# lars-frogner/Impact

Measured on AMD Instinct MI355X. Metric: voxels stepped/sec + remesh tris/sec, 512^3 grid, 1/2/4/8 MI355X, higher is better.
Workload: dtype i8 voxels, f32 SDF/mesh arithmetic, f64 moments; 1 GPU; config-2 SDF asteroid x2.05 -> 502^3 grid = 512^3 stored voxels (32768 chunks); parallelism=single GPU, voxels_per_gpu=134217728, regions=1, triangles=1813104

## Files before the change

### impact_amd/csrc/derive.hip

```cpp
#include "device_common.hpp"
#include "chunk_passes.hpp"
#include "table_roles.hpp"
#include "many.hpp"

#ifndef IVX_POL_SWEEP_PLANES
#define IVX_POL_SWEEP_PLANES IVX_ST_WT
#endif
#ifndef IVX_DERIVE_WAVES
#define IVX_DERIVE_WAVES 6
#endif

namespace {

struct DeriveParams {
    uint32_t cx, cy, cz;
};

__device__ __forceinline__ uint32_t row_mask(uint4 s) {
    uint32_t w[4] = {s.x, s.y, s.z, s.w};
    uint32_t m = 0;
#pragma unroll
    for (int q = 0; q < 4; ++q) m |= ((((w[q] >> 7) & 0x01010101u) * 0x00204081u >> 21) & 0xFu) << (4 * q);
    return m;
}
// ... 8 lines not shown
    GridView g;
    ivx_chunk_info* info;
    uint32_t* bbox;
    uint32_t* mesh_counts;
    uint8_t* chunk_class;
    uint8_t* touch;
    uint32_t* rparent;
    uint32_t* work_counts;
    uint32_t* next_work_count;
    uint32_t* active_list;
    ivx_roles::PresetArgs preset;
    uint32_t defer_ghost, pad_;
    unsigned long long* tick;
};
__device__ __forceinline__ void chunk_settle(const GridView& g, const ChunkPreArgs& a, uint32_t chunk, const ivx_chunk_info& own) {
    const uint32_t gen = own.gen_kind;
    const bool solid = gen == KIND_UNIFORM;
    ivx_chunk_info rec = own;
    rec.kind = (uint8_t)gen;
    rec.flags = 0;
    rec.face_dist = solid ? 0x555 : 0;
    rec.uniform_type = solid ? (own.kind == KIND_NONUNIFORM ? g.type[(size_t)chunk * IVX_CHUNK_VOXELS] : own.uniform_type) : (uint8_t)0;
    rec.region_count = solid ? 1 : 0;
    rec.boundary_region_count = solid ? 1 : 0;
    a.info[chunk] = rec;
    a.bbox[chunk] = solid ? (0x80000000u | (15u << 4) | (15u << 12) | (15u << 20)) : 0u;
    a.mesh_counts[2 * chunk] = 0;
    a.mesh_counts[2 * chunk + 1] = 0;
    a.touch[chunk] = solid ? 7 : 0;
    if (solid) a.rparent[(size_t)chunk * 256] = chunk * 256u;
}
__device__ __forceinline__ void chunk_pre_body(const ChunkPreArgs& a, uint32_t bid, uint32_t) {
    const GridView& g = a.g;
    ivx_chunk_info* __restrict__ info = a.info;
    uint32_t* __restrict__ bbox = a.bbox;
    uint32_t* __restrict__ mesh_counts = a.mesh_counts;
    uint8_t* __restrict__ chunk_class = a.chunk_class;
    uint8_t* __restrict__ touch = a.touch;
    uint32_t* __restrict__ rparent = a.rparent;
    uint32_t* __restrict__ work_counts = a.work_counts;
    uint32_t* __restrict__ next_work_count = a.next_work_count;
    uint32_t* __restrict__ active_list = a.active_list;
    __shared__ uint32_t s_w[4];
    __shared__ uint32_t s_base;
    const uint32_t tid = threadIdx.x, lane = tid & 63u, wave = tid >> 6;
    ivx_roles::role_preset(a.preset, bid * 256u + tid);
    if (bid == 0 && tid == 0) next_work_count[0] = 0u;
    const uint32_t n_chunks = g.cx * g.cy * g.cz;
    const uint32_t chunk = bid * 256u + tid;
    const bool live = chunk < n_chunks;
    bool settled = false, pending = false;
    if (live) {
        const ivx_chunk_info own = info[chunk];
        const uint32_t gen = own.gen_kind;
// ... 135 lines not shown
    int8_t* sdf_rw;
    uint8_t* type_rw;
    uint8_t* flags_out;
    ivx_chunk_info* info;
    uint32_t* bbox;
    uint8_t* touch;
    uint16_t* signs;
    uint8_t* kface_out;
    const uint32_t* work_counts;
    uint32_t* active_list;
    const uint32_t* list_in;
    DeriveFused fz;
    uint32_t signs_type, x_part;
    DeriveBox box;
    unsigned long long* tick;
};
template <bool SIGNS>
__device__ __forceinline__ void derive_body(const DeriveArgs& a_, uint32_t bid_, uint32_t nb_) {
    const GridView& g = a_.g;
    int8_t* __restrict__ sdf_rw = a_.sdf_rw;
    uint8_t* __restrict__ type_rw = a_.type_rw;
    uint8_t* __restrict__ flags_out = a_.flags_out;
    ivx_chunk_info* __restrict__ info = a_.info;
    uint32_t* __restrict__ bbox = a_.bbox;
    uint8_t* __restrict__ touch = a_.touch;
    uint16_t* __restrict__ signs = a_.signs;
    uint8_t* __restrict__ kface_out = a_.kface_out;
    const uint32_t* __restrict__ work_counts = a_.work_counts;
    uint32_t* __restrict__ active_list = a_.active_list;
    const uint32_t* __restrict__ list_in = a_.list_in;
// ... 685 lines not shown
            ci_.flags = 0;
            ci_.face_dist = 0x555;
            ci_.uniform_type = (uint8_t)utype;
        } else {
            ci_.flags = 0;
            ci_.face_dist = 0;
        }
        info[chunk] = ci_;
    }
    IVX_TW(g, li, 5);
    ivx_wave_lds_sync();
    }
}
__global__ __launch_bounds__(256) __attribute__((amdgpu_waves_per_eu(IVX_DERIVE_WAVE_WAVES, 8))) void k_derive_wave(DeriveArgs a) {
    ivx_stage_stamp(a.tick);
    derive_wave_body(a);
}

struct ListRebuildArgs {
    GridView g;
    const ivx_chunk_info* info;
    uint32_t* work_counts;
    uint32_t* next_work_count;
    uint32_t* active_list;
    uint32_t* mesh_counts;
};
__device__ __forceinline__ void list_rebuild_body(const ListRebuildArgs& a, uint32_t bid, uint32_t) {
    const GridView& g = a.g;
    const ivx_chunk_info* __restrict__ info = a.info;
    uint32_t* __restrict__ work_counts = a.work_counts;
// ... 131 lines not shown
    g->planes_compact = 0;
    return IVX_OK;
}

ivx_roles::PresetArgs ivx_preset_args(ivx_grid* g, uint32_t groups) {
    const uint32_t n_groups = (g->n_chunks + 255u) / 256u;
    ivx_roles::PresetArgs a;
    a.groups = groups;
    a.rscalar = g->rscalar;
    a.sn_sums = g->group_sums + n_groups;
    a.n_sn = IVX_SN_GROUP_WORDS * n_groups;
    a.eval_count = g->samp_len ? g->samp_len + g->n_chunks : nullptr;
    return a;
}

int ivx_launch_step_preset(ivx_grid* g, uint32_t groups) {
    if (!groups) return IVX_OK;
    const ivx_roles::PresetArgs a = ivx_preset_args(g, groups);
    IVX_KLAUNCH(k_step_preset, dim3((a.n_sn + 255u) / 256u), dim3(256), 0, g->ctx->stream, a);
    IVX_HIP_CHECK(hipGetLastError());
    g->scratch_dirty &= ~groups;
    return IVX_OK;
}

#ifdef IVX_DERIVE_DEBUG
static void derive_debug_mask() {
    static bool done = false;
    if (done) return;
    done = true;
    const char* e = getenv("IVX_DERIVE_SKIP");
// ... 7 lines not shown
#endif
    GridView v = ivx_view(g);
    DeriveFused fz;
    fz.parts = parts;
    fz.x_off = g->x_off;
    fz.labels = g->llabel;
    fz.rparent = g->rparent;
    fz.rscalar = g->rscalar;
    fz.multi_list = g->ccl_scratch;
    fz.dens = g->dens_dev;
    fz.chunk_moments = g->chunk_moments;
    if ((parts & IVX_PART_REGIONS) && !(preset_groups & IVX_SCRATCH_REGIONS) && (g->scratch_dirty & IVX_SCRATCH_REGIONS))
        IVX_HIP_CHECK(ivx_memset_async(g->rscalar, 0, 16 * sizeof(uint32_t), g->ctx->stream));
    if (parts & IVX_PART_REGIONS) g->scratch_dirty |= IVX_SCRATCH_REGIONS;
    g->bbox_valid = 1;
    uint32_t* next_count = ivx_wc(g);
    g->wc_cur ^= 1u;
    const uint32_t roll = ((g->scratch_dirty & IVX_SCRATCH_EVAL) && g->samp_len) ? IVX_SCRATCH_EVAL_ROLL : 0u;
    ChunkPreArgs face_settle;
    {
        ChunkPreArgs pa;
        memset(&pa, 0, sizeof(pa));
        pa.g = v, pa.info = g->info, pa.bbox = g->chunk_bbox, pa.mesh_counts = g->chunk_counts, pa.chunk_class = g->chunk_class, pa.touch = g->chunk_touch;
        pa.rparent = g->rparent, pa.work_counts = ivx_wc(g), pa.next_work_count = next_count, pa.active_list = g->active_list;
        pa.preset = ivx_preset_args(g, preset_groups | roll);
        if (g->ghost_event && g->ghost_split && ivx_has_interior_planes(g)) pa.defer_ghost = 1u;
        const uint32_t blocks = (g->n_chunks + 255u) / 256u;
        pa.tick = g->timing.take(ivx_many_recording());
        if (!ivx_many_try(g->ctx, g, IVX_MK_CHUNK_PRE, blocks, pa)) IVX_KLAUNCH(k_chunk_pre, dim3(blocks), dim3(256), 0, g->ctx->stream, pa);
        face_settle = pa;
        face_settle.tick = nullptr;
    }
    g->scratch_dirty &= ~preset_groups;
    if (roll) g->scratch_dirty &= ~IVX_SCRATCH_EVAL;
    uint32_t derive_grid = ivx_list_grid(g);
    if (g->last_active) {
        const uint32_t per_round = (uint32_t)g->ctx->n_cu * 32u;
        const uint32_t each = (g->last_active + per_round / 2u) / per_round > 1u ? (g->last_active + per_round / 2u) / per_round : 1u;
        derive_grid = (g->last_active + each - 1u) / each;
        const uint32_t lo = (g->n_chunks + 255u) / 256u;
        if (derive_grid < lo) derive_grid = lo;
    }
    DeriveArgs da = derive_args(g, v, fz);
    if (g->signs_current) da.signs_type = (uint32_t)g->signs_type;
    uint32_t wave_grid;
    {
        const uint32_t per_round = (uint32_t)g->ctx->n_cu * 4u * IVX_DERIVE_WAVE_WAVES;
        const uint32_t n = g->last_active ? g->last_active : per_round;
        const uint32_t each = (n + per_round / 2u) / per_round > 1u ? (n + per_round / 2u) / per_round : 1u;
        wave_grid = ((n + each - 1u) / each + 3u) / 4u;
    }
    auto sweep = [&](uint32_t x_part) {
        da.x_part = x_part;
        da.tick = g->timing.take(ivx_many_recording());
        if (g->signs_current) {
            if (ivx_many_try(g->ctx, g, IVX_MK_DERIVE_SIGNS, derive_grid, da)) return;
            if (x_part == IVX_XPART_ALL && v.ghost_sdf[0] == nullptr && v.ghost_sdf[1] == nullptr)
                IVX_KLAUNCH(k_derive_wave, dim3(wave_grid), dim3(256), 0, g->ctx->stream, da);
            else
// ... 90 lines not shown
```

### impact_amd/csrc/ivx_api.hip

```cpp
#include <algorithm>
#include <array>
#include <functional>
#include <cmath>
#include <chrono>
#include <cstring>
#include <new>
#include <type_traits>
#include <vector>

#include "ivx_host.hpp"

static thread_local char g_error[512] = "";

void ivx_set_error(const char* fmt, ...) {
    va_list ap;
    va_start(ap, fmt);
    vsnprintf(g_error, sizeof(g_error), fmt, ap);
    va_end(ap);
}

namespace {

int ensure_host_scratch(ivx_grid* g, size_t bytes) {
    if (g->host_scratch_bytes >= bytes) return IVX_OK;
// ... 402 lines not shown
    if (which == 0 || which == 1 || which == 4) ivx_planes_touched(g);
    switch (which) {
        case 0: return g->sdf;
        case 1: return g->type;
        case 2: return g->flags;
        case 3: return g->llabel;
        case 4: return g->info;
        case 5: return g->rparent;
#ifdef IVX_WG_TRACE
        case 6: return g->chunk_moments;
#endif
        case 7: return g->samp_len;
        case 8: return g->samp_ops;
        case 10: return g->sn_hard;
        case 9: return ivx_sn_hard_count(g);
        default: return nullptr;
    }
}

int ivx_sdf_sample(ivx_grid* g, const ivx_sdf_processed_node* nodes, size_t n_nodes, uint32_t stack_size, const uint32_t grid_shape[3],
                   const float shifted_grid_center[3], uint8_t voxel_type) {
    IVX_REQUIRE(g && grid_shape && shifted_grid_center, IVX_ERR_INVALID, "ivx_sdf_sample: null argument");
    IVX_REQUIRE(n_nodes == 0 || nodes, IVX_ERR_INVALID, "ivx_sdf_sample: null node array");
    for (int d = 0; d < 3; ++d) {
        const uint32_t cap = (d == 0 ? g->gx : g->cc[d]) * 16u;
        IVX_REQUIRE(grid_shape[d] <= cap, IVX_ERR_INVALID, "ivx_sdf_sample: grid shape %u exceeds the chunk grid (%u voxels) along axis %d", grid_shape[d], cap, d);
    }
    int depth = 0, max_depth = 0;
    for (size_t i = 0; i < n_nodes; ++i) {
        const uint32_t k = nodes[i].kind;
// ... 688 lines not shown
```

### impact_amd/csrc/ivx_internal.hpp

```cpp
#pragma once
#include <hip/hip_runtime.h>

#include <cstdarg>
#include <cstdint>
#include <cstdio>
#include <cstring>

#include "../../include/impact_voxel_hip.h"
#include "many.hpp"
#include "stage_clock.hpp"

static inline hipError_t ivx_memset_async(void* p, int v, size_t n, hipStream_t s) {
    (void)ivx_many_break();
    return hipMemsetAsync(p, v, n, s);
}
static inline hipError_t ivx_memcpy_async(void* d, const void* src, size_t n, hipMemcpyKind k, hipStream_t s) {
    (void)ivx_many_break();
    return hipMemcpyAsync(d, src, n, k, s);
}
static inline hipError_t ivx_stream_sync(hipStream_t s) {
    (void)ivx_many_break();
    return hipStreamSynchronize(s);
}
static inline hipError_t ivx_memcpy_sync(void* d, const void* src, size_t n, hipMemcpyKind k) {
// ... 100 lines not shown
    uint32_t* rcompid;
    uint32_t* rscalar;
    uint32_t* ccl_scratch;
    uint32_t* sn_list;
    uint32_t* group_sums;
    uint32_t* sn_walk;
    uint32_t* sn_hard;
    uint32_t region_count;
    int regions_valid;
    uint32_t* work_counts;
    uint32_t wc_cur;
    uint32_t scratch_dirty;
    uint32_t* occ_part;
    uint32_t* active_list;
    uint8_t* chunk_class;
    uint8_t* kface;
    uint16_t* chunk_signs;
    uint8_t* chunk_touch;
    double* chunk_moments;
    uint32_t last_active;
    int planes_compact;
    int signs_current;
    uint8_t signs_type;
    int active_list_stale;
    int regions_labelled_locally;
    struct ivx_edit_state* edit;
    uint32_t post1_needs_box[12];
    const uint32_t* post1_needs_touched;
    uint32_t* post1_needs_out;
    int early_needs_on;
// ... 244 lines not shown
}

static inline bool ivx_has_interior_planes(const ivx_grid* g) { return (int)g->cc[0] - (g->has_ghost[0] ? 1 : 0) - (g->has_ghost[1] ? 1 : 0) > 0; }
static inline uint32_t* ivx_wc(const ivx_grid* g) { return g->work_counts + g->wc_cur; }
static inline void ivx_voxels_replaced(ivx_grid* g) { g->mesh_valid = g->mesh_built = g->occ_ref_valid = g->bbox_valid = g->regions_valid = 0; }
static inline void ivx_planes_touched(ivx_grid* g) {
    g->signs_current = 0;
    g->needs_current = 0;
}
#define IVX_SCRATCH_EVAL_ROLL 8u
#define IVX_SCRATCH_REGIONS 1u
#define IVX_SCRATCH_SN 2u
#define IVX_SN_TAIL_WORDS 288u
#define IVX_SN_GROUP_WORDS 32u
#define IVX_SCRATCH_EVAL 4u

static inline GridView ivx_view(const ivx_grid* g) {
    GridView v;
    v.cx = g->cc[0];
    v.cy = g->cc[1];
    v.cz = g->cc[2];
    v.sdf = g->sdf;
    v.type = g->type;
    v.signs = g->chunk_signs;
    v.kface = g->kface;
#ifdef IVX_WG_TRACE
    v.trace = reinterpret_cast<unsigned long long*>(g->chunk_moments);
#endif
    v.info = g->info;
    for (int s = 0; s < 2; ++s) {
// ... 91 lines not shown
```

### impact_amd/csrc/sdf_sample.hip

```cpp
#include <cmath>

#include "ivx_internal.hpp"
#include "device_common.hpp"
#include "noise.hpp"
#include "table_roles.hpp"

namespace {

struct V3 {
    float x, y, z;
};
__device__ __forceinline__ V3 mk(float x, float y, float z) { return V3{x, y, z}; }
__device__ __forceinline__ V3 add(V3 a, V3 b) { return {a.x + b.x, a.y + b.y, a.z + b.z}; }
__device__ __forceinline__ V3 sub(V3 a, V3 b) { return {a.x - b.x, a.y - b.y, a.z - b.z}; }
__device__ __forceinline__ V3 scale(V3 a, float s) { return {a.x * s, a.y * s, a.z * s}; }
__device__ __forceinline__ float dot3(V3 a, V3 b) { return (a.x * b.x + a.y * b.y) + a.z * b.z; }
__device__ __forceinline__ float sqrt_rn(float x) {
    const float s = __builtin_amdgcn_sqrtf(x);
    const float s_dn = __uint_as_float(__float_as_uint(s) - 1u), s_up = __uint_as_float(__float_as_uint(s) + 1u);
    const float r_dn = __builtin_fmaf(-s_dn, s, x), r_up = __builtin_fmaf(-s_up, s, x);
    float r = r_dn <= 0.0f ? s_dn : s;
    r = r_up > 0.0f ? s_up : r;
    return r;
}
// ... 682 lines not shown
    }
    if (wv != 0u) continue;
    IVX_TP(p, sb, 2);
    const float lo = p.n_nodes ? s_lo[0][tid] : 1000.0f, hi = p.n_nodes ? s_hi[0][tid] : 1000.0f;
    float out = __uint_as_float(0x7FC00000u);
    if (p.n_nodes == 0u) cmask = 1u;
    if (cmask & 1u) out = lo;
    else if (lo >= 2.54f + 0.02f) out = 1000.0f;
    else if (hi <= -2.56f - 0.02f) out = -1000.0f;
    if (poisoned) out = __uint_as_float(0x7FC00000u), pos = OP_CAP + 1u;
    if (oi >= p.shape[0] || oj >= p.shape[1] || ok >= p.shape[2]) out = 1000.0f;
    bool to_fill = false;
    if (mine) {
        prog_len[chunk] = pos <= OP_CAP ? pos : OP_OVERFLOW;
        bool settled = false;
        if (out == out) {
            const int sdq = sd_from_f32(out);
            const bool whole = oi + 16u <= p.shape[0] && oj + 16u <= p.shape[1] && ok + 16u <= p.shape[2];
            const bool is_void = sdq > SD_VOID_LIMIT;
            const bool is_uniform = whole && sdq == -128;
            if (is_void || is_uniform) {
                ivx_chunk_info rec;
                rec.kind = rec.gen_kind = (uint8_t)(is_void ? KIND_VOID : KIND_UNIFORM);
                rec.flags = 0;
                rec.uniform_type = is_uniform ? (uint8_t)p.voxel_type : (uint8_t)0;
                rec.face_dist = 0;
                rec.region_count = 0;
                rec.boundary_region_count = 0;
                info_out[chunk] = rec;
                settled = true;
            } else {
                to_fill = true;
            }
        }
        if (ahead && !settled) {
            ivx_chunk_info rec;
            rec.kind = rec.gen_kind = AHEAD_OPEN;
            rec.flags = rec.uniform_type = 0;
            rec.face_dist = 0;
            rec.region_count = rec.boundary_region_count = 0;
            info_out[chunk] = rec;
        }
    }
    static_assert(PRE_T == 64, "the list appends below assume one wave (the first of the block) doing them");
    {
        const unsigned long long below = (1ull << tid) - 1ull;
        const bool ev = mine && (out != out || to_fill);
        const uint32_t need = pos <= OP_CAP ? (uint32_t)s_need[0][tid] : max(p.stack_size, 2u);
        const uint32_t cls = NOISE ? 2u : (need <= 1u ? 0u : (need == 2u ? 1u : 2u));
// ... 338 lines not shown
        }
    }
}

#ifndef IVX_EVAL_WAVES
#define IVX_EVAL_WAVES 8
#endif
template <int MODE, bool NOISE = false>
__global__ __launch_bounds__(256) __attribute__((amdgpu_waves_per_eu(IVX_EVAL_WAVES, 8))) void k_sdf_eval(SampleParams p, const uint32_t* __restrict__ eval_count, const uint32_t* __restrict__ eval_list,
                                                  const uint32_t* __restrict__ long_count, const uint32_t* __restrict__ first_count,
                                                  const uint32_t* __restrict__ first_list, uint32_t list_len, uint32_t scratch_off,
                                                  const uint32_t* __restrict__ prog_len, const uint2* __restrict__ prog_ops,
                                                  const ivx_sdf_processed_node* __restrict__ nodes, int8_t* __restrict__ sdf_out,
                                                  uint8_t* __restrict__ type_out, ivx_chunk_info* __restrict__ info_out,
                                                  uint16_t* __restrict__ signs_out, uint8_t* __restrict__ kface_out,
                                                  const ivx_chunk_info* __restrict__ shadow, uint32_t n_chunks, ivx_roles::PresetArgs preset) {
    extern __shared__ float stack[];
    ivx_stage_stamp(p.tick);
    constexpr bool TRIM = MODE == 1;
    const uint32_t tid = threadIdx.x;
    const uint32_t ti = tid >> 4, tj = tid & 15u;
    if (shadow) {
        for (uint32_t gid = blockIdx.x * 256u + tid; gid < max(preset.n_sn, 32u); gid += gridDim.x * 256u) ivx_roles::role_preset(preset, gid);
        const uint32_t each = (n_chunks + gridDim.x - 1u) / gridDim.x;
        const uint32_t c0 = blockIdx.x * each, c1 = min(c0 + each, n_chunks);
        for (uint32_t c = c0 + tid; c < c1; c += 256u) {
            const ivx_chunk_info r = shadow[c];
            if (r.kind != AHEAD_OPEN) info_out[c] = r;
        }
    }
    const uint32_t n_first = first_count ? first_count[0] : 0u;
    const uint32_t n_eval = n_first + eval_count[0];
    const uint32_t n_long = long_count ? long_count[0] : eval_count[0];
    for (uint32_t li = blockIdx.x; li < n_eval; li += gridDim.x) {
    __syncthreads();
    IVX_TE(p, li, 0);
    const uint32_t lj = li - n_first;
    const uint32_t chunk = li < n_first ? first_list[li] : eval_list[lj < n_long ? lj : list_len - 1u - (lj - n_long)];
    const uint32_t ck = chunk % p.cz, cj = (chunk / p.cz) % p.cy, ci = chunk / (p.cz * p.cy);
    const uint32_t oi = (ci + p.x_off) * 16u, oj = cj * 16u, ok = ck * 16u;
    int sd[16];

    const V3 origin_root = sub(mk((float)oi, (float)oj, (float)ok), mk(p.shifted_center[0], p.shifted_center[1], p.shifted_center[2]));
    const Box block{origin_root, add(origin_root, mk(16.0f, 16.0f, 16.0f))};

    float cv = 0.0f;
    float r15 = 0.0f;
    uint32_t tail = 0u;
    float tail_c = 0.0f, tail_s = 0.0f, tail_q = 0.0f;
// ... 283 lines not shown
        ci_.face_dist = 0;
        ci_.region_count = 0;
        ci_.boundary_region_count = 0;
        info[chunk] = ci_;
    }
}

__global__ __launch_bounds__(256) void k_voxel_types_eval(TypeNoiseParams p, uint8_t* __restrict__ out) {
    const uint32_t tid = threadIdx.x;
    *reinterpret_cast<uint4*>(out + (size_t)tid * 16) =
        type_noise_row(p.shifted_center[0], p.shifted_center[1], p.shifted_center[2], tid >> 4, tid & 15u, p.n, p.noise_freq, p.type_freq, p.seed);
}

}

int ivx_sampler_buffers(ivx_grid* g) {
    if (g->samp_ops) return IVX_OK;
    IVX_HIP_CHECK(hipMalloc(reinterpret_cast<void**>(&g->samp_len), sizeof(uint32_t) * (4 * (size_t)g->n_chunks + 16)));
    IVX_HIP_CHECK(ivx_memset_async(g->samp_len + g->n_chunks, 0, 16 * sizeof(uint32_t), g->ctx->stream));
    IVX_HIP_CHECK(hipMalloc(reinterpret_cast<void**>(&g->samp_ops), sizeof(uint2) * (size_t)OP_CAP * g->n_chunks));
    return IVX_OK;
}

static int ivx_aux_stream(ivx_ctx* c, hipStream_t* out) {
    if (!c->aux_stream) IVX_HIP_CHECK(hipStreamCreateWithFlags(&c->aux_stream, hipStreamNonBlocking));
    *out = c->aux_stream;
    return IVX_OK;
}
static int ivx_sampler_ahead_buffers(ivx_grid* g, hipStream_t aux) {
    if (!g->ahead_events_ready) {
        IVX_HIP_CHECK(hipEventCreateWithFlags(&g->ahead_go, hipEventDisableTiming));
        IVX_HIP_CHECK(hipEventCreateWithFlags(&g->ahead_done, hipEventDisableTiming));
        g->ahead_events_ready = 1;
    }
    if (g->samp_ops_alt) return IVX_OK;
    IVX_HIP_CHECK(hipMalloc(reinterpret_cast<void**>(&g->samp_len_alt), sizeof(uint32_t) * (4 * (size_t)g->n_chunks + 16)));
    IVX_HIP_CHECK(hipMemsetAsync(g->samp_len_alt + g->n_chunks, 0, 16 * sizeof(uint32_t), aux));
    g->alt_eval_dirty = 0;
    IVX_HIP_CHECK(hipMalloc(reinterpret_cast<void**>(&g->samp_ops_alt), sizeof(uint2) * (size_t)OP_CAP * g->n_chunks));
    IVX_HIP_CHECK(hipMalloc(reinterpret_cast<void**>(&g->info_shadow), 2 * sizeof(ivx_chunk_info) * (size_t)g->n_chunks));
    return IVX_OK;
}
int ivx_sampler_ahead_cancel(ivx_grid* g) {
    if (!g->ahead_pending) return IVX_OK;
    g->ahead_pending = 0;
    g->alt_eval_dirty = 1;
    IVX_HIP_CHECK(hipEventSynchronize(g->ahead_done));
    return IVX_OK;
}
void ivx_sampler_ahead_free(ivx_grid* g) {
    (void)ivx_sampler_ahead_cancel(g);
    if (g->samp_len_alt) (void)hipFree(g->samp_len_alt);
    if (g->samp_ops_alt) (void)hipFree(g->samp_ops_alt);
    if (g->info_shadow) (void)hipFree(g->info_shadow);
    g->samp_len_alt = nullptr, g->samp_ops_alt = nullptr, g->info_shadow = nullptr;
    if (g->ahead_events_ready) {
        (void)hipEventDestroy(g->ahead_go);
        (void)hipEventDestroy(g->ahead_done);
        g->ahead_events_ready = 0;
    }
}

ivx_roles::PresetArgs ivx_preset_args(ivx_grid* g, uint32_t groups);

int ivx_launch_sdf_sample(ivx_grid* g, const ivx_sdf_processed_node* d_nodes, uint32_t n_nodes, uint32_t stack_size,
                          const uint32_t shape[3], const float shifted_center[3], uint8_t voxel_type, uint32_t preset_groups,
                          bool resident_program, bool noise) {
    SampleParams p;
    p.cx = g->cc[0];
    p.cy = g->cc[1];
    p.cz = g->cc[2];
    p.x_off = g->x_off;
    for (int d = 0; d < 3; ++d) {
        p.shape[d] = shape[d];
        p.shifted_center[d] = shifted_center[d];
    }
    p.n_nodes = n_nodes;
    p.stack_size = stack_size;
// ... 78 lines not shown
    g->planes_compact = 1;
    {
        auto fit = [&](uint32_t n) {
            const uint32_t cap = g->n_chunks < 16384u ? g->n_chunks : 16384u;
            if (!known || n == 0u) return cap;
            const uint32_t each = (n + cap - 1u) / cap;
            return (n + each - 1u) / each;
        };
        const ivx_chunk_info* shadow = consume ? g->info_shadow + (size_t)g->shadow_sel * g->n_chunks : nullptr;
        const ivx_roles::PresetArgs no_presets = ivx_preset_args(g, 0u), first_presets = ivx_preset_args(g, consume ? host_presets : 0u);
        auto take_shadow = [&]() {
            const ivx_chunk_info* s_ = shadow;
            shadow = nullptr;
            return s_;
        };
        uint32_t* const list0 = eval_list;
        uint32_t* const list1 = eval_list + (size_t)g->n_chunks;
        if (launch2) {
            const uint32_t scratch_off = IVX_CHUNK_VOXELS;
            const ivx_chunk_info* sh = take_shadow();
            p.tick = g->timing.take(ivx_many_recording());
            IVX_KLAUNCH(k_sdf_eval<2>, dim3(fit(g->eval_len[0])), dim3(256), (size_t)(scratch_off + 64u) * sizeof(float), g->ctx->stream, p, eval_count + 0, list0,
                               eval_count + 3, nullptr, nullptr, g->n_chunks, scratch_off, g->samp_len, ops, d_nodes, g->sdf, g->type, g->info, g->chunk_signs, g->kface,
                               sh, g->n_chunks, sh ? first_presets : no_presets);
        }
        if (launch1) {
            const uint32_t scratch_off = IVX_CHUNK_VOXELS + 15u * 256u;
            const ivx_chunk_info* sh = take_shadow();
            p.tick = g->timing.take(ivx_many_recording());
            if (merge01)
                IVX_KLAUNCH(k_sdf_eval<1>, dim3(fit(g->eval_len[0] + g->eval_len[1])), dim3(256), (size_t)(scratch_off + 64u) * sizeof(float), g->ctx->stream, p, eval_count + 0, list0,
                                   eval_count + 3, eval_count + 1, list1, g->n_chunks, scratch_off, g->samp_len, ops, d_nodes, g->sdf, g->type, g->info, g->chunk_signs, g->kface,
                                   sh, g->n_chunks, sh ? first_presets : no_presets);
            else
                IVX_KLAUNCH(k_sdf_eval<1>, dim3(fit(g->eval_len[1])), dim3(256), (size_t)(scratch_off + 64u) * sizeof(float), g->ctx->stream, p, eval_count + 1, list1,
                                   nullptr, nullptr, nullptr, g->n_chunks, scratch_off, g->samp_len, ops, d_nodes, g->sdf, g->type, g->info, g->chunk_signs, g->kface,
                                   sh, g->n_chunks, sh ? first_presets : no_presets);
        }
        if (launch0) {
            const uint32_t lv = stack_size ? stack_size : 1u;
            const uint32_t scratch_off = lv * IVX_CHUNK_VOXELS - 16u;
            const ivx_chunk_info* sh = take_shadow();
            p.tick = g->timing.take(ivx_many_recording());
            if (noise)
                IVX_KLAUNCH((k_sdf_eval<0, true>), dim3(fit(g->eval_len[2])), dim3(256), (size_t)lv * IVX_CHUNK_VOXELS * sizeof(float), g->ctx->stream, p, eval_count + 2,
                                   eval_list + 2 * (size_t)g->n_chunks, nullptr, nullptr, nullptr, g->n_chunks, scratch_off, g->samp_len, ops, d_nodes, g->sdf, g->type, g->info,
                                   g->chunk_signs, g->kface, sh, g->n_chunks, sh ? first_presets : no_presets);
            else
                IVX_KLAUNCH(k_sdf_eval<0>, dim3(fit(g->eval_len[2])), dim3(256), (size_t)lv * IVX_CHUNK_VOXELS * sizeof(float), g->ctx->stream, p, eval_count + 2,
                                   eval_list + 2 * (size_t)g->n_chunks, nullptr, nullptr, nullptr, g->n_chunks, scratch_off, g->samp_len, ops, d_nodes, g->sdf, g->type, g->info,
                                   g->chunk_signs, g->kface, sh, g->n_chunks, sh ? first_presets : no_presets);
        }
    }
    const bool type_noise = g->vt_n >= 2u;
    if (type_noise) {
        TypeNoiseParams tp;
        tp.cy = g->cc[1], tp.cz = g->cc[2], tp.x_off = g->x_off, tp.n = g->vt_n;
        for (int d = 0; d < 3; ++d) tp.shifted_center[d] = shifted_center[d];
        tp.noise_freq = g->vt_noise_freq, tp.type_freq = g->vt_type_freq, tp.seed = g->vt_seed;
        IVX_KLAUNCH(k_voxel_type_noise, dim3(g->n_chunks), dim3(256), 0, g->ctx->stream, tp, g->sdf, g->type, g->info, g->chunk_signs, g->kface);
    }
    IVX_HIP_CHECK(hipGetLastError());
    g->ahead_wanted = (g->ahead_on && ahead_fits) ? 1 : 0;
    if (g->ahead_wanted && g->ahead_unordered_ok) {
        const int rc_a = ivx_sampler_launch_ahead(g, false);
        if (rc_a) return rc_a;
// ... 143 lines not shown
```

### impact_amd/csrc/step_api.hip

```cpp
#include "ivx_host.hpp"

extern "C" {

static const bool g_stage_timing_events = getenv("IVX_STAGE_TIMING_EVENTS") && atoi(getenv("IVX_STAGE_TIMING_EVENTS")) == 1;
namespace {
struct StageRt {
    hipStream_t s;
    int make_events(ivx_stage_timing& t) {
        if (t.ev_ready) return IVX_OK;
        for (int i = 0; i < 2 * IVX_N_TIMED_STAGES; ++i) IVX_HIP_CHECK(hipEventCreate(reinterpret_cast<hipEvent_t*>(&t.ev[i])));
        t.ev_ready = 1;
        return IVX_OK;
    }
    int make_ticks(ivx_stage_timing& t) {
        if (!t.tick_dev) {
            IVX_HIP_CHECK(hipMalloc(reinterpret_cast<void**>(&t.tick_dev), IVX_TICK_WORDS * sizeof(unsigned long long)));
            IVX_HIP_CHECK(hipMemset(t.tick_dev, 0, IVX_TICK_WORDS * sizeof(unsigned long long)));
        }
        if (!t.tick_host) {
            IVX_HIP_CHECK(hipHostMalloc(reinterpret_cast<void**>(&t.tick_host), IVX_TICK_WORDS * sizeof(unsigned long long), hipHostMallocMapped));
            memset(t.tick_host, 0, IVX_TICK_WORDS * sizeof(unsigned long long));
            IVX_HIP_CHECK(hipHostGetDevicePointer(reinterpret_cast<void**>(&t.tick_host_dev), t.tick_host, 0));
        }
        return IVX_OK;
// ... 53 lines not shown
        }
        if (stages & IVX_STAGE_SAMPLE) preset_in_sample = need | ahead;
        else if (stages & IVX_STAGE_DERIVE) preset_in_derive = need | ahead;
        else if ((rc = ivx_launch_step_preset(g, need & ~fresh))) return rc;
        g->preset_fresh = ahead;
    }
    const uint32_t fused_parts = (stages & IVX_STAGE_DERIVE) ? (((stages & IVX_STAGE_REGIONS) ? IVX_PART_REGIONS : 0u) |
                                                                 ((stages & IVX_STAGE_INERTIA) ? IVX_PART_MOMENTS : 0u))
                                                              : 0u;
    const uint32_t post = back ? stages & (IVX_STAGE_OCCUPIED | IVX_STAGE_REGIONS | IVX_STAGE_REMESH | IVX_STAGE_INERTIA) : 0u;
    const bool standalone_first = ((post & IVX_STAGE_REGIONS) && !(fused_parts & IVX_PART_REGIONS) && !g->regions_labelled_locally) ||
                                  ((post & IVX_STAGE_INERTIA) && !(fused_parts & IVX_PART_MOMENTS));
    ivx_stage_timing& clk = g->timing;
    StageRt rt{s};
    if ((rc = clk.begin(rt, ivx_stage_call{part, g_stage_timing_events, slab_record != nullptr, ivx_step_assign_fits(g), standalone_first, ivx_many_recording()}))) return rc;
    if (front && (stages & IVX_STAGE_SAMPLE)) {
        if ((rc = clk.open(rt, 0))) return rc;
        if ((rc = ivx_launch_sdf_sample(g, g->prog_nodes, g->prog_n, g->prog_stack, g->prog_shape, g->prog_center, g->prog_type, preset_in_sample, true,
                                        g->prog_noise != 0))) return rc;
        if ((rc = clk.close(rt, 0))) return rc;
        g->eval_len_pending = 1;
        ivx_voxels_replaced(g);
    }
    if (front && (stages & IVX_STAGE_DERIVE)) {
        if ((rc = clk.open(rt, 1))) return rc;
        if ((rc = ivx_launch_derive(g, fused_parts, preset_in_derive))) return rc;
        if ((rc = clk.close(rt, 1))) return rc;
        if (g->eval_len_pending == 1) g->eval_len_pending = 2;
    }
    if (post) {
        if ((stages & IVX_STAGE_REGIONS) && !(fused_parts & IVX_PART_REGIONS)) {
            if (!g->regions_labelled_locally && (rc = ivx_launch_ccl_local_only(g))) return rc;
        }
        if ((stages & IVX_STAGE_INERTIA) && !(fused_parts & IVX_PART_MOMENTS))
            if ((rc = ivx_launch_inertia_dense(g))) return rc;
// ... 254 lines not shown
```

### impact_amd/csrc/table_roles.hpp

```cpp
#pragma once
#include "ivx_internal.hpp"

namespace ivx_roles {

__device__ __forceinline__ void role_occupied_partial(uint32_t bid, uint32_t cx, uint32_t cy, uint32_t cz, const uint32_t* __restrict__ bbox,
                                                      uint32_t* __restrict__ occ_part) {
    __shared__ uint32_t s_red[4][12];
    const uint32_t tid = threadIdx.x, lane = tid & 63u, wave = tid >> 6;
    const uint32_t n = cx * cy * cz;
    const uint32_t c = bid * 256u + tid;
    const uint32_t p = c < n ? bbox[c] : 0u;
    uint32_t v[12];
#pragma unroll
    for (int q = 0; q < 12; ++q) v[q] = q < 6 ? 0xFFFFFFFFu : 0u;
    if (p & 0x80000000u) {
        const uint32_t ck = c % cz, cj = (c / cz) % cy, ci = c / (cz * cy);
        const uint32_t cc[3] = {ci, cj, ck};
#pragma unroll
        for (int d = 0; d < 3; ++d) {
            v[d] = cc[d];
            v[6 + d] = cc[d] + 1;
            v[3 + d] = cc[d] * 16u + ((p >> (8 * d)) & 15u);
            v[9 + d] = cc[d] * 16u + ((p >> (8 * d + 4)) & 15u) + 1u;
        }
// ... 127 lines not shown
    uint32_t* sn_sums;
    uint32_t n_sn;
    uint32_t* eval_count;
};
__device__ __forceinline__ void role_preset(const PresetArgs& a, uint32_t gid) {
    if ((a.groups & IVX_SCRATCH_REGIONS) && gid < 16u) a.rscalar[gid] = 0u;
    if ((a.groups & IVX_SCRATCH_SN) && gid < a.n_sn) a.sn_sums[gid] = 0u;
    if ((a.groups & IVX_SCRATCH_SN) && gid < 9u) a.sn_sums[a.n_sn + 32u * gid] = 0u;
    if ((a.groups & IVX_SCRATCH_EVAL) && gid < 5u && a.eval_count) a.eval_count[gid] = 0u;
    if ((a.groups & IVX_SCRATCH_EVAL_ROLL) && gid < 5u && a.eval_count) {
        a.eval_count[8u + gid] = a.eval_count[gid];
        a.eval_count[gid] = 0u;
    }
}

}
```

Measured before the change: 890.7 billion voxels/s.

## Fuse active-list sweep into SDF evaluator launch via per-chunk verdict bytes

The SDF sampler now writes a per-chunk verdict byte (eval/void/uniform) and, when conditions allow, appends extra blocks to the evaluator launch that settle fully-surrounded uniform chunks and build the derive active list. The derive pass then skips its separate chunk-pre kernel and folds the eval-count preset roll into the derive-wave kernel. The aim is to remove a standalone kernel launch and a full pass over chunk info between sampling and derive. In exchange it adds state flags that couple the sample and derive stages, a larger sampler buffer, and a state check that raises an error if the preconditions do not hold.

```diff
diff --git a/impact_amd/csrc/derive.hip b/impact_amd/csrc/derive.hip
--- a/impact_amd/csrc/derive.hip
+++ b/impact_amd/csrc/derive.hip
@@ -46,30 +46,13 @@
     unsigned long long* tick;
 };
 __device__ __forceinline__ void chunk_settle(const GridView& g, const ChunkPreArgs& a, uint32_t chunk, const ivx_chunk_info& own) {
-    const uint32_t gen = own.gen_kind;
-    const bool solid = gen == KIND_UNIFORM;
-    ivx_chunk_info rec = own;
-    rec.kind = (uint8_t)gen;
-    rec.flags = 0;
-    rec.face_dist = solid ? 0x555 : 0;
-    rec.uniform_type = solid ? (own.kind == KIND_NONUNIFORM ? g.type[(size_t)chunk * IVX_CHUNK_VOXELS] : own.uniform_type) : (uint8_t)0;
-    rec.region_count = solid ? 1 : 0;
-    rec.boundary_region_count = solid ? 1 : 0;
-    a.info[chunk] = rec;
-    a.bbox[chunk] = solid ? (0x80000000u | (15u << 4) | (15u << 12) | (15u << 20)) : 0u;
-    a.mesh_counts[2 * chunk] = 0;
-    a.mesh_counts[2 * chunk + 1] = 0;
-    a.touch[chunk] = solid ? 7 : 0;
-    if (solid) a.rparent[(size_t)chunk * 256] = chunk * 256u;
+    const uint8_t utype = own.gen_kind == KIND_UNIFORM ? (own.kind == KIND_NONUNIFORM ? g.type[(size_t)chunk * IVX_CHUNK_VOXELS] : own.uniform_type) : (uint8_t)0;
+    ivx_roles::chunk_settle_words(a.info, a.bbox, a.mesh_counts, a.touch, a.rparent, chunk, own, utype);
 }
 __device__ __forceinline__ void chunk_pre_body(const ChunkPreArgs& a, uint32_t bid, uint32_t) {
     const GridView& g = a.g;
     ivx_chunk_info* __restrict__ info = a.info;
-    uint32_t* __restrict__ bbox = a.bbox;
-    uint32_t* __restrict__ mesh_counts = a.mesh_counts;
     uint8_t* __restrict__ chunk_class = a.chunk_class;
-    uint8_t* __restrict__ touch = a.touch;
-    uint32_t* __restrict__ rparent = a.rparent;
     uint32_t* __restrict__ work_counts = a.work_counts;
     uint32_t* __restrict__ next_work_count = a.next_work_count;
     uint32_t* __restrict__ active_list = a.active_list;
@@ -235,6 +218,7 @@
     uint32_t signs_type, x_part;
     DeriveBox box;
     unsigned long long* tick;
+    ivx_roles::PresetArgs preset;
 };
 template <bool SIGNS>
 __device__ __forceinline__ void derive_body(const DeriveArgs& a_, uint32_t bid_, uint32_t nb_) {
@@ -950,6 +934,7 @@
 }
 __global__ __launch_bounds__(256) __attribute__((amdgpu_waves_per_eu(IVX_DERIVE_WAVE_WAVES, 8))) void k_derive_wave(DeriveArgs a) {
     ivx_stage_stamp(a.tick);
+    ivx_roles::role_preset(a.preset, blockIdx.x * 256u + threadIdx.x);
     derive_wave_body(a);
 }
 
@@ -1111,6 +1096,18 @@
     return a;
 }
 
+ivx_roles::SweepListArgs ivx_sweep_list_args(ivx_grid* g, const uint8_t* verdict) {
+    ivx_roles::SweepListArgs a;
+    a.verdict = verdict;
+    a.bbox = g->chunk_bbox, a.mesh_counts = g->chunk_counts, a.chunk_class = g->chunk_class, a.touch = g->chunk_touch, a.rparent = g->rparent;
+    a.next_work_count = ivx_wc(g);
+    g->wc_cur ^= 1u;
+    a.work_counts = ivx_wc(g);
+    a.active_list = g->active_list;
+    g->sweep_list_made = 1;
+    return a;
+}
+
 int ivx_launch_step_preset(ivx_grid* g, uint32_t groups) {
     if (!groups) return IVX_OK;
     const ivx_roles::PresetArgs a = ivx_preset_args(g, groups);
@@ -1148,11 +1145,16 @@
         IVX_HIP_CHECK(ivx_memset_async(g->rscalar, 0, 16 * sizeof(uint32_t), g->ctx->stream));
     if (parts & IVX_PART_REGIONS) g->scratch_dirty |= IVX_SCRATCH_REGIONS;
     g->bbox_valid = 1;
+    const bool listed = g->sweep_list_made != 0;
+    g->sweep_list_made = 0;
+    IVX_REQUIRE(!listed || (preset_groups == 0u && g->signs_current && !g->ghost_event && v.ghost_sdf[0] == nullptr && v.ghost_sdf[1] == nullptr && !ivx_many_recording()),
+                IVX_ERR_STATE, "ivx_launch_derive: the active list came with the evaluator launch, but the sweep's wave form does not apply");
     uint32_t* next_count = ivx_wc(g);
-    g->wc_cur ^= 1u;
+    if (!listed) g->wc_cur ^= 1u;
     const uint32_t roll = ((g->scratch_dirty & IVX_SCRATCH_EVAL) && g->samp_len) ? IVX_SCRATCH_EVAL_ROLL : 0u;
     ChunkPreArgs face_settle;
-    {
+    memset(&face_settle, 0, sizeof(face_settle));
+    if (!listed) {
         ChunkPreArgs pa;
         memset(&pa, 0, sizeof(pa));
         pa.g = v, pa.info = g->info, pa.bbox = g->chunk_bbox, pa.mesh_counts = g->chunk_counts, pa.chunk_class = g->chunk_class, pa.touch = g->chunk_touch;
@@ -1177,6 +1179,7 @@
     }
     DeriveArgs da = derive_args(g, v, fz);
     if (g->signs_current) da.signs_type = (uint32_t)g->signs_type;
+    da.preset = ivx_preset_args(g, listed ? roll : 0u);
     uint32_t wave_grid;
     {
         const uint32_t per_round = (uint32_t)g->ctx->n_cu * 4u * IVX_DERIVE_WAVE_WAVES;
diff --git a/impact_amd/csrc/ivx_api.hip b/impact_amd/csrc/ivx_api.hip
--- a/impact_amd/csrc/ivx_api.hip
+++ b/impact_amd/csrc/ivx_api.hip
@@ -440,6 +440,13 @@
         case 8: return g->samp_ops;
         case 10: return g->sn_hard;
         case 9: return ivx_sn_hard_count(g);
+        case 11: return g->chunk_signs;
+        case 12: return g->kface;
+        case 13: return g->chunk_bbox;
+        case 14: return g->chunk_touch;
+        case 15: return g->chunk_counts;
+        case 16: return ivx_wc(g);
+        case 17: return g->active_list;
         default: return nullptr;
     }
 }
diff --git a/impact_amd/csrc/ivx_internal.hpp b/impact_amd/csrc/ivx_internal.hpp
--- a/impact_amd/csrc/ivx_internal.hpp
+++ b/impact_amd/csrc/ivx_internal.hpp
@@ -138,6 +138,7 @@
     uint32_t* occ_part;
     uint32_t* active_list;
     uint8_t* chunk_class;
+    int sweep_list_want, sweep_list_made;
     uint8_t* kface;
     uint16_t* chunk_signs;
     uint8_t* chunk_touch;
@@ -412,6 +413,9 @@
 #define IVX_SN_TAIL_WORDS 288u
 #define IVX_SN_GROUP_WORDS 32u
 #define IVX_SCRATCH_EVAL 4u
+#define IVX_PRE_EVAL 0u
+#define IVX_PRE_VOID 1u
+#define IVX_PRE_UNIFORM 2u
 
 static inline GridView ivx_view(const ivx_grid* g) {
     GridView v;
diff --git a/impact_amd/csrc/sdf_sample.hip b/impact_amd/csrc/sdf_sample.hip
--- a/impact_amd/csrc/sdf_sample.hip
+++ b/impact_amd/csrc/sdf_sample.hip
@@ -720,6 +720,7 @@
     if (mine) {
         prog_len[chunk] = pos <= OP_CAP ? pos : OP_OVERFLOW;
         bool settled = false;
+        uint32_t verdict = IVX_PRE_EVAL;
         if (out == out) {
             const int sdq = sd_from_f32(out);
             const bool whole = oi + 16u <= p.shape[0] && oj + 16u <= p.shape[1] && ok + 16u <= p.shape[2];
@@ -735,10 +736,12 @@
                 rec.boundary_region_count = 0;
                 info_out[chunk] = rec;
                 settled = true;
+                verdict = is_void ? IVX_PRE_VOID : IVX_PRE_UNIFORM;
             } else {
                 to_fill = true;
             }
         }
+        reinterpret_cast<uint8_t*>(eval_list + 3u * (size_t)list_stride)[chunk] = (uint8_t)verdict;
         if (ahead && !settled) {
             ivx_chunk_info rec;
             rec.kind = rec.gen_kind = AHEAD_OPEN;
@@ -1107,25 +1110,33 @@
                                                   const ivx_sdf_processed_node* __restrict__ nodes, int8_t* __restrict__ sdf_out,
                                                   uint8_t* __restrict__ type_out, ivx_chunk_info* __restrict__ info_out,
                                                   uint16_t* __restrict__ signs_out, uint8_t* __restrict__ kface_out,
-                                                  const ivx_chunk_info* __restrict__ shadow, uint32_t n_chunks, ivx_roles::PresetArgs preset) {
+                                                  const ivx_chunk_info* __restrict__ shadow, uint32_t n_chunks, ivx_roles::PresetArgs preset,
+                                                  uint32_t sweep_blocks, ivx_roles::SweepListArgs sweep) {
     extern __shared__ float stack[];
     ivx_stage_stamp(p.tick);
     constexpr bool TRIM = MODE == 1;
     const uint32_t tid = threadIdx.x;
     const uint32_t ti = tid >> 4, tj = tid & 15u;
+    const uint32_t n_blocks = gridDim.x - sweep_blocks;
+    if (blockIdx.x >= n_blocks) {
+        ivx_roles::role_sweep_list(sweep, blockIdx.x - n_blocks, p.cx, p.cy, p.cz, info_out, shadow, reinterpret_cast<uint32_t*>(stack));
+        return;
+    }
     if (shadow) {
-        for (uint32_t gid = blockIdx.x * 256u + tid; gid < max(preset.n_sn, 32u); gid += gridDim.x * 256u) ivx_roles::role_preset(preset, gid);
-        const uint32_t each = (n_chunks + gridDim.x - 1u) / gridDim.x;
-        const uint32_t c0 = blockIdx.x * each, c1 = min(c0 + each, n_chunks);
-        for (uint32_t c = c0 + tid; c < c1; c += 256u) {
-            const ivx_chunk_info r = shadow[c];
-            if (r.kind != AHEAD_OPEN) info_out[c] = r;
+        for (uint32_t gid = blockIdx.x * 256u + tid; gid < max(preset.n_sn, 32u); gid += n_blocks * 256u) ivx_roles::role_preset(preset, gid);
+        if (!sweep_blocks) {
+            const uint32_t each = (n_chunks + n_blocks - 1u) / n_blocks;
+            const uint32_t c0 = blockIdx.x * each, c1 = min(c0 + each, n_chunks);
+            for (uint32_t c = c0 + tid; c < c1; c += 256u) {
+                const ivx_chunk_info r = shadow[c];
+                if (r.kind != AHEAD_OPEN) info_out[c] = r;
+            }
         }
     }
     const uint32_t n_first = first_count ? first_count[0] : 0u;
     const uint32_t n_eval = n_first + eval_count[0];
     const uint32_t n_long = long_count ? long_count[0] : eval_count[0];
-    for (uint32_t li = blockIdx.x; li < n_eval; li += gridDim.x) {
+    for (uint32_t li = blockIdx.x; li < n_eval; li += n_blocks) {
     __syncthreads();
     IVX_TE(p, li, 0);
     const uint32_t lj = li - n_first;
@@ -1439,9 +1450,10 @@
 
 }
 
+static size_t samp_len_bytes(const ivx_grid* g) { return sizeof(uint32_t) * (4 * (size_t)g->n_chunks + 16) + (((size_t)g->n_chunks + 3u) & ~(size_t)3u); }
 int ivx_sampler_buffers(ivx_grid* g) {
     if (g->samp_ops) return IVX_OK;
-    IVX_HIP_CHECK(hipMalloc(reinterpret_cast<void**>(&g->samp_len), sizeof(uint32_t) * (4 * (size_t)g->n_chunks + 16)));
+    IVX_HIP_CHECK(hipMalloc(reinterpret_cast<void**>(&g->samp_len), samp_len_bytes(g)));
     IVX_HIP_CHECK(ivx_memset_async(g->samp_len + g->n_chunks, 0, 16 * sizeof(uint32_t), g->ctx->stream));
     IVX_HIP_CHECK(hipMalloc(reinterpret_cast<void**>(&g->samp_ops), sizeof(uint2) * (size_t)OP_CAP * g->n_chunks));
     return IVX_OK;
@@ -1459,7 +1471,7 @@
         g->ahead_events_ready = 1;
     }
     if (g->samp_ops_alt) return IVX_OK;
-    IVX_HIP_CHECK(hipMalloc(reinterpret_cast<void**>(&g->samp_len_alt), sizeof(uint32_t) * (4 * (size_t)g->n_chunks + 16)));
+    IVX_HIP_CHECK(hipMalloc(reinterpret_cast<void**>(&g->samp_len_alt), samp_len_bytes(g)));
     IVX_HIP_CHECK(hipMemsetAsync(g->samp_len_alt + g->n_chunks, 0, 16 * sizeof(uint32_t), aux));
     g->alt_eval_dirty = 0;
     IVX_HIP_CHECK(hipMalloc(reinterpret_cast<void**>(&g->samp_ops_alt), sizeof(uint2) * (size_t)OP_CAP * g->n_chunks));
@@ -1487,6 +1499,7 @@
 }
 
 ivx_roles::PresetArgs ivx_preset_args(ivx_grid* g, uint32_t groups);
+ivx_roles::SweepListArgs ivx_sweep_list_args(ivx_grid* g, const uint8_t* verdict);
 
 int ivx_launch_sdf_sample(ivx_grid* g, const ivx_sdf_processed_node* d_nodes, uint32_t n_nodes, uint32_t stack_size,
                           const uint32_t shape[3], const float shifted_center[3], uint8_t voxel_type, uint32_t preset_groups,
@@ -1595,42 +1608,57 @@
             shadow = nullptr;
             return s_;
         };
+        uint32_t sweep_blocks = 0u;
+        ivx_roles::SweepListArgs sweep_args;
+        memset(&sweep_args, 0, sizeof(sweep_args));
+        if (g->sweep_list_want && resident_program && (launch0 || launch1 || launch2)) {
+            sweep_args = ivx_sweep_list_args(g, reinterpret_cast<const uint8_t*>(eval_list + 3 * (size_t)g->n_chunks));
+            sweep_blocks = (g->n_chunks + 255u) / 256u;
+        }
+        auto take_sweep = [&]() {
+            const uint32_t b_ = sweep_blocks;
+            sweep_blocks = 0u;
+            return b_;
+        };
         uint32_t* const list0 = eval_list;
         uint32_t* const list1 = eval_list + (size_t)g->n_chunks;
         if (launch2) {
             const uint32_t scratch_off = IVX_CHUNK_VOXELS;
             const ivx_chunk_info* sh = take_shadow();
+            const uint32_t sb = take_sweep();
             p.tick = g->timing.take(ivx_many_recording());
-            IVX_KLAUNCH(k_sdf_eval<2>, dim3(fit(g->eval_len[0])), dim3(256), (size_t)(scratch_off + 64u) * sizeof(float), g->ctx->stream, p, eval_count + 0, list0,
+            IVX_KLAUNCH(k_sdf_eval<2>, dim3(fit(g->eval_len[0]) + sb), dim3(256), (size_t)(scratch_off + 64u) * sizeof(float), g->ctx->stream, p, eval_count + 0, list0,
                                eval_count + 3, nullptr, nullptr, g->n_chunks, scratch_off, g->samp_len, ops, d_nodes, g->sdf, g->type, g->info, g->chunk_signs, g->kface,
-                               sh, g->n_chunks, sh ? first_presets : no_presets);
+                               sh, g->n_chunks, sh ? first_presets : no_presets, sb, sweep_args);
         }
         if (launch1) {
             const uint32_t scratch_off = IVX_CHUNK_VOXELS + 15u * 256u;
             const ivx_chunk_info* sh = take_shadow();
+            const uint32_t sb = take_sweep();
             p.tick = g->timing.take(ivx_many_recording());
             if (merge01)
-                IVX_KLAUNCH(k_sdf_eval<1>, dim3(fit(g->eval_len[0] + g->eval_len[1])), dim3(256), (size_t)(scratch_off + 64u) * sizeof(float), g->ctx->stream, p, eval_count + 0, list0,
+                IVX_KLAUNCH(k_sdf_eval<1>, dim3(fit(g->eval_len[0] + g->eval_len[1]) + sb), dim3(256), (size_t)(scratch_off + 64u) * sizeof(float), g->ctx->stream, p, eval_count + 0, list0,
                                    eval_count + 3, eval_count + 1, list1, g->n_chunks, scratch_off, g->samp_len, ops, d_nodes, g->sdf, g->type, g->info, g->chunk_signs, g->kface,
-                                   sh, g->n_chunks, sh ? first_presets : no_presets);
+                                   sh, g->n_chunks, sh ? first_presets : no_presets, sb, sweep_args);
             else
-                IVX_KLAUNCH(k_sdf_eval<1>, dim3(fit(g->eval_len[1])), dim3(256), (size_t)(scratch_off + 64u) * sizeof(float), g->ctx->stream, p, eval_count + 1, list1,
+                IVX_KLAUNCH(k_sdf_eval<1>, dim3(fit(g->eval_len[1]) + sb), dim3(256), (size_t)(scratch_off + 64u) * sizeof(float), g->ctx->stream, p, eval_count + 1, list1,
                                    nullptr, nullptr, nullptr, g->n_chunks, scratch_off, g->samp_len, ops, d_nodes, g->sdf, g->type, g->info, g->chunk_signs, g->kface,
-                                   sh, g->n_chunks, sh ? first_presets : no_presets);
+                                   sh, g->n_chunks, sh ? first_presets : no_presets, sb, sweep_args);
         }
         if (launch0) {
             const uint32_t lv = stack_size ? stack_size : 1u;
             const uint32_t scratch_off = lv * IVX_CHUNK_VOXELS - 16u;
             const ivx_chunk_info* sh = take_shadow();
+            const uint32_t sb = take_sweep();
             p.tick = g->timing.take(ivx_many_recording());
             if (noise)
-                IVX_KLAUNCH((k_sdf_eval<0, true>), dim3(fit(g->eval_len[2])), dim3(256), (size_t)lv * IVX_CHUNK_VOXELS * sizeof(float), g->ctx->stream, p, eval_count + 2,
+                IVX_KLAUNCH((k_sdf_eval<0, true>), dim3(fit(g->eval_len[2]) + sb), dim3(256), (size_t)lv * IVX_CHUNK_VOXELS * sizeof(float), g->ctx->stream, p, eval_count + 2,
                                    eval_list + 2 * (size_t)g->n_chunks, nullptr, nullptr, nullptr, g->n_chunks, scratch_off, g->samp_len, ops, d_nodes, g->sdf, g->type, g->info,
-                                   g->chunk_signs, g->kface, sh, g->n_chunks, sh ? first_presets : no_presets);
+                                   g->chunk_signs, g->kface, sh, g->n_chunks, sh ? first_presets : no_presets, sb, sweep_args);
             else
-                IVX_KLAUNCH(k_sdf_eval<0>, dim3(fit(g->eval_len[2])), dim3(256), (size_t)lv * IVX_CHUNK_VOXELS * sizeof(float), g->ctx->stream, p, eval_count + 2,
+                IVX_KLAUNCH(k_sdf_eval<0>, dim3(fit(g->eval_len[2]) + sb), dim3(256), (size_t)lv * IVX_CHUNK_VOXELS * sizeof(float), g->ctx->stream, p, eval_count + 2,
                                    eval_list + 2 * (size_t)g->n_chunks, nullptr, nullptr, nullptr, g->n_chunks, scratch_off, g->samp_len, ops, d_nodes, g->sdf, g->type, g->info,
-                                   g->chunk_signs, g->kface, sh, g->n_chunks, sh ? first_presets : no_presets);
+                                   g->chunk_signs, g->kface, sh, g->n_chunks, sh ? first_presets : no_presets, sb, sweep_args);
         }
     }
     const bool type_noise = g->vt_n >= 2u;
diff --git a/impact_amd/csrc/step_api.hip b/impact_amd/csrc/step_api.hip
--- a/impact_amd/csrc/step_api.hip
+++ b/impact_amd/csrc/step_api.hip
@@ -91,11 +91,17 @@
     ivx_stage_timing& clk = g->timing;
     StageRt rt{s};
     if ((rc = clk.begin(rt, ivx_stage_call{part, g_stage_timing_events, slab_record != nullptr, ivx_step_assign_fits(g), standalone_first, ivx_many_recording()}))) return rc;
+    static const bool sweep_list_off = getenv("IVX_SWEEP_LIST") && atoi(getenv("IVX_SWEEP_LIST")) == 0;
+    g->sweep_list_made = 0;
+    g->sweep_list_want = (!sweep_list_off && front && (stages & IVX_STAGE_SAMPLE) && (stages & IVX_STAGE_DERIVE) && !g->has_ghost[0] && !g->has_ghost[1] && !g->ghost_event &&
+                          !ivx_many_recording() && g->vt_n < 2u && !g->prog_noise)
+                             ? 1 : 0;
     if (front && (stages & IVX_STAGE_SAMPLE)) {
         if ((rc = clk.open(rt, 0))) return rc;
         if ((rc = ivx_launch_sdf_sample(g, g->prog_nodes, g->prog_n, g->prog_stack, g->prog_shape, g->prog_center, g->prog_type, preset_in_sample, true,
                                         g->prog_noise != 0))) return rc;
         if ((rc = clk.close(rt, 0))) return rc;
+        g->sweep_list_want = 0;
         g->eval_len_pending = 1;
         ivx_voxels_replaced(g);
     }
diff --git a/impact_amd/csrc/table_roles.hpp b/impact_amd/csrc/table_roles.hpp
--- a/impact_amd/csrc/table_roles.hpp
+++ b/impact_amd/csrc/table_roles.hpp
@@ -165,4 +165,75 @@
     }
 }
 
-}
+__device__ __forceinline__ void chunk_settle_words(ivx_chunk_info* __restrict__ info, uint32_t* __restrict__ bbox, uint32_t* __restrict__ mesh_counts,
+                                                   uint8_t* __restrict__ touch, uint32_t* __restrict__ rparent, uint32_t chunk, const ivx_chunk_info& own,
+                                                   uint8_t utype) {
+    const uint32_t gen = own.gen_kind;
+    const bool solid = gen == KIND_UNIFORM;
+    ivx_chunk_info rec = own;
+    rec.kind = (uint8_t)gen;
+    rec.flags = 0;
+    rec.face_dist = solid ? 0x555 : 0;
+    rec.uniform_type = solid ? utype : (uint8_t)0;
+    rec.region_count = solid ? 1 : 0;
+    rec.boundary_region_count = solid ? 1 : 0;
+    info[chunk] = rec;
+    bbox[chunk] = solid ? (0x80000000u | (15u << 4) | (15u << 12) | (15u << 20)) : 0u;
+    mesh_counts[2 * chunk] = 0;
+    mesh_counts[2 * chunk + 1] = 0;
+    touch[chunk] = solid ? 7 : 0;
+    if (solid) rparent[(size_t)chunk * 256] = chunk * 256u;
+}
+
+struct SweepListArgs {
+    const uint8_t* verdict;
+    uint32_t* bbox;
+    uint32_t* mesh_counts;
+    uint8_t* chunk_class;
+    uint8_t* touch;
+    uint32_t* rparent;
+    uint32_t* work_counts;
+    uint32_t* next_work_count;
+    uint32_t* active_list;
+};
+__device__ __forceinline__ void role_sweep_list(const SweepListArgs& a, uint32_t bid, uint32_t cx, uint32_t cy, uint32_t cz, ivx_chunk_info* __restrict__ info,
+                                                const ivx_chunk_info* __restrict__ shadow, uint32_t* s_words) {
+    const uint32_t tid = threadIdx.x, lane = tid & 63u, wave = tid >> 6;
+    if (bid == 0 && tid == 0) a.next_work_count[0] = 0u;
+    const uint32_t n_chunks = cx * cy * cz;
+    const uint32_t chunk = bid * 256u + tid;
+    const bool live = chunk < n_chunks;
+    bool settled = false;
+    if (live) {
+        const uint8_t* __restrict__ verdict = a.verdict;
+        const uint32_t v = verdict[chunk];
+        if (v != IVX_PRE_EVAL) {
+            settled = v == IVX_PRE_VOID;
+            if (v == IVX_PRE_UNIFORM) {
+                const uint32_t ck = chunk % cz, cj = (chunk / cz) % cy, ci = chunk / (cz * cy);
+                if (ci > 0u && cj > 0u && ck > 0u && ci + 1u < cx && cj + 1u < cy && ck + 1u < cz) {
+                    const uint32_t sx = cy * cz, sy = cz;
+                    settled = verdict[chunk - sx] == IVX_PRE_UNIFORM && verdict[chunk + sx] == IVX_PRE_UNIFORM && verdict[chunk - sy] == IVX_PRE_UNIFORM &&
+                              verdict[chunk + sy] == IVX_PRE_UNIFORM && verdict[chunk - 1u] == IVX_PRE_UNIFORM && verdict[chunk + 1u] == IVX_PRE_UNIFORM;
+                }
+            }
+            const ivx_chunk_info own = shadow ? shadow[chunk] : info[chunk];
+            if (settled) chunk_settle_words(info, a.bbox, a.mesh_counts, a.touch, a.rparent, chunk, own, own.uniform_type);
+            else if (shadow) info[chunk] = own;
+        }
+        a.chunk_class[chunk] = settled ? 1 : 0;
+    }
+    const bool active = live && !settled;
+    const unsigned long long bal = __ballot(active);
+    if (lane == 0) s_words[wave] = (uint32_t)__popcll(bal);
+    __syncthreads();
+    if (tid == 0) s_words[4] = atomicAdd(&a.work_counts[0], (s_words[0] + s_words[1]) + (s_words[2] + s_words[3]));
+    __syncthreads();
+    if (active) {
+        uint32_t off = s_words[4] + (uint32_t)__popcll(bal & ((1ull << lane) - 1ull));
+        for (uint32_t w = 0; w < wave; ++w) off += s_words[w];
+        a.active_list[off] = chunk;
+    }
+}
+
+}
```

Result: faster. 911.1 billion voxels/s (median of 5 runs) (+2.3%).
